# gongaa/SlidingWindowDecoder

Measured on AMD Instinct MI355X. Metric: sliding windows decoded/s, [[144,12,12]] BB p=0.003, higher is better.
Workload: dtype f64

## Files before the change

include/swd.h:

```cpp
#ifndef SWD_H
#define SWD_H

#include <stdint.h>

#ifdef __cplusplus
extern "C" {
#endif

#define SWD_ABI_VERSION 4

enum {
    SWD_EXIT_PRE = 0,
    SWD_EXIT_POST = 1,
    SWD_EXIT_OSD = 2,
    SWD_EXIT_FAIL_SET = 3,
    SWD_EXIT_FAIL_PEEL = 4,
    SWD_EXIT_NO_OSD = 5,
    SWD_EXIT_SCHED_FAULT = 6
};
#define SWD_STATUS_CONVERGE 0x100

typedef struct swd_graph_desc {
    int32_t m, n, nnz;
    const int32_t *row_ptr;
// ... 146 lines not shown
typedef struct swd_rolling swd_rolling;
swd_rolling *swd_pipeline_rolling_create(swd_pipeline *pl, int32_t max_shots);
void swd_pipeline_rolling_destroy(swd_rolling *s);
int swd_pipeline_rolling_begin(swd_rolling *s, int32_t B);
int swd_pipeline_rolling_push(swd_rolling *s, int32_t nrows, const uint8_t *det_rows, int32_t max_windows, uint8_t *faults,
                              int32_t *stats, double *min_pm, int64_t *first, int32_t *count);
int swd_pipeline_rolling_push_dev(swd_rolling *s, int32_t nrows, const uint8_t *det_rows, int64_t stride, int32_t max_windows,
                                  uint8_t *faults, int32_t *stats, double *min_pm, int64_t *first, int32_t *count, void *stream);
int swd_pipeline_rolling_finish(swd_rolling *s, int32_t nrows, const uint8_t *final_rows, uint8_t *faults, int32_t *stats,
                                double *min_pm, int32_t *shot_result);
int swd_pipeline_rolling_finish_dev(swd_rolling *s, int32_t nrows, const uint8_t *final_rows, int64_t stride, uint8_t *faults,
                                    int32_t *stats, double *min_pm, int32_t *shot_result, void *stream);
int swd_pipeline_rolling_state(swd_rolling *s, int64_t *rows_received, int64_t *windows_done, int32_t *frame_fill, int32_t *info,
                               int64_t *device_bytes);


int swd_pipeline_set_profiling(swd_pipeline *pl, int32_t on);
int swd_pipeline_get_profile(swd_pipeline *pl, int32_t B, int64_t *out);
int swd_pipeline_set_timing(swd_pipeline *pl, int32_t on);
int swd_pipeline_get_timing(swd_pipeline *pl, double *total_ms, int64_t *launches);

int swd_diag_occupy(int device, int32_t blocks, int32_t threads, int32_t lds_bytes, int32_t microseconds, void *stream);

#ifdef __cplusplus
}
#endif
#endif
```

slidingwindowdecoder_amd/_lib.py:

```python
from __future__ import annotations

import ctypes as C
import os

_HERE = os.path.dirname(os.path.abspath(__file__))
LIB_PATH = os.path.join(_HERE, os.environ.get("SWD_LIB", "libswd_hip.so"))
_lib = None


class GraphDesc(C.Structure):
    _fields_ = [("m", C.c_int32), ("n", C.c_int32), ("nnz", C.c_int32),
                ("row_ptr", C.c_void_p), ("col_idx", C.c_void_p), ("channel_probs", C.c_void_p)]


class WindowDesc(C.Structure):
    _fields_ = [("graph", GraphDesc), ("row0", C.c_int32), ("col0", C.c_int32), ("commit", C.c_int32),
                ("reserved", C.c_int32)]


class OsdwParams(C.Structure):
    _fields_ = [("pre_max_iter", C.c_int32), ("post_max_iter", C.c_int32),
                ("ms_scaling_factor", C.c_double), ("new_n", C.c_int32),
                ("osd_method", C.c_int32), ("osd_order", C.c_int32)]

# ... 57 lines not shown
    ("swd_pipeline_session_push_dev", C.c_int, [_vp, _i32, _vp, _i64, C.POINTER(_i32), C.POINTER(_i32), _vp]),
    ("swd_pipeline_session_window", C.c_int, [_vp, _i32, _vp, _vp, _vp]),
    ("swd_pipeline_session_finish", C.c_int, [_vp, _vp, _vp, _vp, _vp]),
    ("swd_pipeline_session_buffers", C.c_int, [_vp, C.POINTER(_vp), C.POINTER(_i64), C.POINTER(_i32), C.POINTER(_i32)]),
    ("swd_pipeline_rolling_create", _vp, [_vp, _i32]),
    ("swd_pipeline_rolling_destroy", None, [_vp]),
    ("swd_pipeline_rolling_begin", C.c_int, [_vp, _i32]),
    ("swd_pipeline_rolling_push", C.c_int, [_vp, _i32, _vp, _i32, _vp, _vp, _vp, C.POINTER(_i64), C.POINTER(_i32)]),
    ("swd_pipeline_rolling_push_dev", C.c_int, [_vp, _i32, _vp, _i64, _i32, _vp, _vp, _vp, C.POINTER(_i64), C.POINTER(_i32), _vp]),
    ("swd_pipeline_rolling_finish", C.c_int, [_vp, _i32, _vp, _vp, _vp, _vp, _vp]),
    ("swd_pipeline_rolling_finish_dev", C.c_int, [_vp, _i32, _vp, _i64, _vp, _vp, _vp, _vp, _vp]),
    ("swd_pipeline_rolling_state", C.c_int, [_vp, C.POINTER(_i64), C.POINTER(_i64), C.POINTER(_i32), C.POINTER(_i32), C.POINTER(_i64)]),
    ("swd_pipeline_status", C.c_int, [_vp, C.POINTER(C.c_uint32)]),
    ("swd_pipeline_set_profiling", C.c_int, [_vp, _i32]),
    ("swd_pipeline_get_profile", C.c_int, [_vp, _i32, _vp]),
    ("swd_pipeline_set_timing", C.c_int, [_vp, _i32]),
    ("swd_pipeline_get_timing", C.c_int, [_vp, C.POINTER(_dbl), C.POINTER(_i64)]),
    ("swd_sampler_create", _vp, [C.POINTER(GraphDesc), C.POINTER(GraphDesc), C.c_int]),
    ("swd_sampler_destroy", None, [_vp]),
    ("swd_sampler_info", C.c_int, [_vp, C.POINTER(_i32), C.POINTER(_i32), C.POINTER(_i32)]),
    ("swd_sampler_sample", C.c_int, [_vp, _i32, C.c_uint64, C.c_uint64, _vp, _vp, _vp]),
    ("swd_sampler_sample_dev", C.c_int, [_vp, _i32, C.c_uint64, C.c_uint64, _vp, _i64, _vp, _vp, _i64, _vp]),
    ("swd_diag_occupy", C.c_int, [C.c_int, _i32, _i32, _i32, _i32, _vp]),
]

STAT_WORDS = 8
STREAM_PACKED, STREAM_NO_STATS = 1, 2
STREAM_NO_DEPENDENCY = C.c_void_p(-1).value


def _preload_torch_hip_runtime():
    import importlib.util
    spec = importlib.util.find_spec("torch")
    if spec is None or not spec.submodule_search_locations:
        return
    libdir = os.path.join(list(spec.submodule_search_locations)[0], "lib")
    for name in ("libhsa-runtime64.so", "libamdhip64.so"):
        path = os.path.join(libdir, name)
        if os.path.exists(path):
            try:
                C.CDLL(path, mode=C.RTLD_GLOBAL)
            except OSError:
                pass


def lib():
# ... 24 lines not shown
```

slidingwindowdecoder_amd/csrc/swd_gdg_kernel.h:

```cpp
#pragma once

#define SWD_GDG_SLOTS 64
#define SWD_GDG_MAXGUESS 160
#define SWD_GDG_MAXSTEP 64
#define SWD_GDG_REC_BYTES (16 + 4 * SWD_GDG_MAXSTEP)
#define SWD_GDG_HDR_BYTES 256

__device__ __forceinline__ uint32_t ag_ld(const uint32_t *p) { return __hip_atomic_load(p, __ATOMIC_RELAXED, __HIP_MEMORY_SCOPE_AGENT); }
__device__ __forceinline__ void ag_st(uint32_t *p, uint32_t v) { __hip_atomic_store(p, v, __ATOMIC_RELAXED, __HIP_MEMORY_SCOPE_AGENT); }
__device__ __forceinline__ void ag_publish_barrier() {
    asm volatile("s_waitcnt vmcnt(0)" ::: "memory");
    __builtin_amdgcn_fence(__ATOMIC_RELEASE, "workgroup");
    __syncthreads();
}

#define SWD_ITEM_UNIT 0u
#define SWD_ITEM_SIDE 1u
#define SWD_ITEM_FINAL 2u
#define SWD_ITEM_NONE 0xFFFFFFFEu
#define SWD_ITEM_EXIT 0xFFFFFFFFu
#define SWD_GDG_ITEM_MAX_WINDOWS 256
#define SWD_GDG_ITEM_MAX_SHOTS (1 << 22)
__device__ __forceinline__ uint32_t item_unit(int b, int wi) { return (SWD_ITEM_UNIT << 30) | ((uint32_t)wi << 22) | (uint32_t)b; }
__device__ __forceinline__ uint32_t item_side(int ctxid, int slot) { return (SWD_ITEM_SIDE << 30) | ((uint32_t)ctxid << 8) | (uint32_t)slot; }
// ... 1281 lines not shown
    for (int i = 0; i < 5; ++i) R.gp[i] = 0;
#endif
    R.t[0] = wall_clock64();
    for (int l = tid; l < m; l += NT) {
        const int d = g.row_deg[l];
        s.cn_val[l] = (int8_t)(synd[g.perm[l]] ? 1 : 0);
        s.cn_deg[l] = (uint8_t)d;
        s.cn_deg0[l] = (uint8_t)d;
        s.livemask[l] = (d >= 64) ? ~0ull : ((1ull << d) - 1ull);
    }
    for (int v = tid; v < n; v += NT) { s.vn_val[v] = -1; s.hard[v] = 0; }
    for (int j = tid; j <= g.K; j += NT) s.jptr[j] = g.jptr[j];
    if (P.zero_hist)
        for (int i = tid; i < 4 * n; i += NT) hist_b[i] = 0.0;
    __syncthreads();
    GdgVC<VF, DM> vc;
    GdgCC<KG> cn;
    vn_cache_load<NT, VF, DM, true>(g, s, n, vc);
    bp_init<VF, DM>(s, vc);
    cn_cache_load<NT, KG, true>(g, s, false, s.ctid < g.m ? s.ctid : -1, 0, 1, cn);
    __syncthreads();
    int it = 0;
    R.conv = 0; R.pm = 0.0; R.pre_it = R.post_it = 0;
    R.live_vn = n; R.live_cn = m; R.live_e = g.E; R.osd_rowadds = 0;
    R.t[1] = wall_clock64();
    R.conv = bp_run<NT, VF, DM, KG, true>(g, P, s, P.pre_iter, n, vc, cn, hist_b, it, P.alpha, false);
    R.pre_it = it; R.total_it = it;
    R.t[2] = wall_clock64();
    if (R.conv) { R.exit_class = SWD_EXIT_PRE; return; }
    if (P.kind == 3) { R.exit_class = SWD_EXIT_NO_OSD; return; }

    uint64_t *key = (uint64_t *)s.scratch;
    uint16_t *idx = (uint16_t *)(s.scratch + L.off_idx);
    __syncthreads();
    if (!par || ENS) gdg_stage_graph<NT>(g_loc, g_in, s);
    for (int v = tid; v < L.npad; v += NT) {
        if (v < n) {
            const double sum = ((hist_b[v] + hist_b[n + v]) + hist_b[2 * n + v]) + hist_b[3 * n + v];
            key[v] = f2key(sum);
            idx[v] = (uint16_t)v;
        } else { key[v] = ~0ull; idx[v] = 0xFFFF; }
    }
    for (int v = tid; v < n; v += NT) G.bp_hard[v] = s.hard[v];
    __syncthreads();
    if (P.max_iter_per_step < 4)
        for (int i = P.max_iter_per_step * n + tid; i < 4 * n; i += NT) hist_b[i] = 0.0;
    int npad2 = 2;
// ... 217 lines not shown
```

slidingwindowdecoder_amd/csrc/swd_graph.h:

```cpp
#pragma once
#include <stdint.h>

#define SWD_MAX_ROW_DEG 64
#define SWD_MAX_COL_DEG 16
#define SWD_MAX_M 1024
#define SWD_MAX_E 65535
#define SWD_PAD_EDGE 0xFFFFFFFFu

struct SwdGraphDev {
    int32_t m, n, E, K, D;
    int32_t new_n, rank, wm;
    const uint16_t *jptr;
    const uint16_t *row_col;
    const uint8_t *row_deg;
    const uint16_t *perm;
    const uint16_t *iperm;
    const uint32_t *vn_edge;
    const uint16_t *vn_row;
    const uint8_t *col_deg;
    const double *llr;
    const uint16_t *vperm;
    const uint32_t *vn_edge_s;
    const double *llr_s;
};

__host__ __device__ inline uint32_t swd_edge_slot(uint32_t e) { return e & 0xFFFFu; }
__host__ __device__ inline uint32_t swd_edge_lane(uint32_t e) { return (e >> 16) & 0x3FFu; }
__host__ __device__ inline uint32_t swd_edge_j(uint32_t e) { return e >> 26; }
```

slidingwindowdecoder_amd/csrc/swd_graph.hip:

```cpp
#include <math.h>
#include <string.h>

#include <mutex>

#include "swd_host.h"

namespace swd {

static thread_local std::string g_err;

void set_error(const char *fmt, ...) {
    char buf[1024];
    va_list ap;
    va_start(ap, fmt);
    vsnprintf(buf, sizeof buf, fmt, ap);
    va_end(ap);
    g_err = buf;
}

const char *last_error() { return g_err.c_str(); }

int gf2_rank(int m, int n, const std::vector<int32_t> &row_ptr, const std::vector<int32_t> &col_idx) {
    const int W = (n + 63) / 64;
    std::vector<uint64_t> rows((size_t)m * W, 0);
// ... 24 lines not shown
            if (col_idx[e] < 0 || col_idx[e] >= n) { set_error("column index out of range in row %d", r); return -1; }
            if (e > row_ptr[r] && col_idx[e] == col_idx[e - 1]) { set_error("duplicate entry in row %d", r); return -1; }
        }
    }
    return 0;
}

void csr_transpose(int m, int n, const double *channel_probs, bool want_r2c, CsrHost &h) {
    const int E = (int)h.col_idx.size();
    h.col_ptr.assign(n + 1, 0);
    h.row_idx.resize(E);
    h.c2r.resize(E);
    std::vector<int32_t> fill(n, 0);
    for (int e = 0; e < E; ++e) h.col_ptr[h.col_idx[e] + 1]++;
    for (int v = 0; v < n; ++v) h.col_ptr[v + 1] += h.col_ptr[v];
    for (int c = 0; c < m; ++c)
        for (int e = h.row_ptr[c]; e < h.row_ptr[c + 1]; ++e) { const int v = h.col_idx[e], k = h.col_ptr[v] + fill[v]++; h.row_idx[k] = c; h.c2r[k] = e; }
    if (want_r2c) {
        h.r2c.resize(E);
        for (int k = 0; k < E; ++k) h.r2c[h.c2r[k]] = k;
    }
    h.llr.resize(n);
    for (int v = 0; v < n; ++v) h.llr[v] = log((1 - channel_probs[v]) / channel_probs[v]);
}

int Graph::build(const swd_graph_desc *g) {
    if (!g || !g->row_ptr || !g->col_idx || !g->channel_probs) { set_error("null graph description"); return -1; }
    m = g->m; n = g->n; E = g->nnz;
    if (m <= 0 || n <= 0 || E <= 0) { set_error("empty check matrix (m=%d n=%d nnz=%d)", m, n, E); return -1; }
    if (g->row_ptr[0] != 0 || g->row_ptr[m] != E) { set_error("row_ptr does not span nnz"); return -1; }
    if (m > SWD_MAX_M) { set_error("m=%d exceeds this build's limit of %d checks", m, SWD_MAX_M); return -1; }
    if (n > 65534) { set_error("n=%d exceeds this build's limit of 65534 columns", n); return -1; }
    if (E > SWD_MAX_E) { set_error("nnz=%d exceeds this build's limit of %d edges", E, SWD_MAX_E); return -1; }
    row_ptr.assign(g->row_ptr, g->row_ptr + m + 1);
    col_idx.assign(g->col_idx, g->col_idx + E);
    if (csr_check_rows(m, n, row_ptr, col_idx)) return -1;
    row_deg.assign(m, 0);
    col_deg.assign(n, 0);
    K = 0; D = 0;
    std::vector<int> cdeg(n, 0);
    for (int r = 0; r < m; ++r) {
        int d = row_ptr[r + 1] - row_ptr[r];
        if (d > SWD_MAX_ROW_DEG) { set_error("row %d has weight %d > %d", r, d, SWD_MAX_ROW_DEG); return -1; }
        if (d == 0) { set_error("row %d is empty: every check needs degree > 0 (osd_window.pyx:117)", r); return -1; }
        K = std::max(K, d);
        for (int e = row_ptr[r]; e < row_ptr[r + 1]; ++e) cdeg[col_idx[e]]++;
    }
    for (int v = 0; v < n; ++v) {
        if (cdeg[v] > SWD_MAX_COL_DEG) { set_error("column %d has weight %d > %d", v, cdeg[v], SWD_MAX_COL_DEG); return -1; }
        D = std::max(D, cdeg[v]);
        col_deg[v] = (uint8_t)cdeg[v];
    }
    perm.resize(m); iperm.resize(m);
    std::vector<int> order(m);
    for (int r = 0; r < m; ++r) order[r] = r;
    std::stable_sort(order.begin(), order.end(), [&](int a, int b) {
        return (row_ptr[a + 1] - row_ptr[a]) > (row_ptr[b + 1] - row_ptr[b]);
    });
    for (int l = 0; l < m; ++l) { perm[l] = (uint16_t)order[l]; iperm[order[l]] = (uint16_t)l; row_deg[l] = (uint8_t)(row_ptr[order[l] + 1] - row_ptr[order[l]]); }
    jptr.assign(K + 1, 0);
    for (int j = 0; j < K; ++j) {
        int cnt = 0;
        for (int l = 0; l < m; ++l) cnt += (row_deg[l] > j);
        jptr[j + 1] = (uint16_t)(jptr[j] + cnt);
    }
    row_col.assign(E, 0);
    col_ptr.assign(n + 1, 0);
    for (int v = 0; v < n; ++v) col_ptr[v + 1] = col_ptr[v] + cdeg[v];
    row_idx.assign(E, 0);
    vn_edge.assign((size_t)std::max(D, 1) * n, SWD_PAD_EDGE);
    vn_row.assign((size_t)std::max(D, 1) * n, 0xFFFF);
    std::vector<int> fill(n, 0);
    for (int r = 0; r < m; ++r) {
        const int l = iperm[r];
        for (int e = row_ptr[r]; e < row_ptr[r + 1]; ++e) {
            const int j = e - row_ptr[r];
            const int v = col_idx[e];
            const int slot = jptr[j] + l;
            row_col[slot] = (uint16_t)v;
            const int k = fill[v]++;
            row_idx[col_ptr[v] + k] = r;
            vn_edge[(size_t)k * n + v] = (uint32_t)slot | ((uint32_t)l << 16) | ((uint32_t)j << 26);
            vn_row[(size_t)k * n + v] = (uint16_t)r;
        }
    }
    llr.resize(n);
    for (int v = 0; v < n; ++v) {
        const double p = g->channel_probs[v];
        llr[v] = log((1 - p) / p);
    }
    {
        std::vector<int> ord(n);
        for (int v = 0; v < n; ++v) ord[v] = v;
        std::stable_sort(ord.begin(), ord.end(), [&](int a, int b) { return (cdeg[a] + 1) / 2 > (cdeg[b] + 1) / 2; });
        vperm.resize(n); llr_s.resize(n);
        vn_edge_s.assign((size_t)std::max(D, 1) * n, SWD_PAD_EDGE);
        for (int i = 0; i < n; ++i) {
            vperm[i] = (uint16_t)ord[i];
            llr_s[i] = llr[ord[i]];
            for (int k = 0; k < D; ++k) vn_edge_s[(size_t)k * n + i] = vn_edge[(size_t)k * n + ord[i]];
        }
    }
    rank = gf2_rank(m, n, row_ptr, col_idx);
    wm = (m + 63) / 64;
    return 0;
}

int Graph::upload() {
    auto al = [](size_t x) { return (x + 255) & ~(size_t)255; };
    size_t o_jptr = 0;
    size_t o_rowcol = al(o_jptr + jptr.size() * 2);
    size_t o_rowdeg = al(o_rowcol + row_col.size() * 2);
    size_t o_perm = al(o_rowdeg + row_deg.size());
    size_t o_iperm = al(o_perm + perm.size() * 2);
    size_t o_vnedge = al(o_iperm + iperm.size() * 2);
    size_t o_vnrow = al(o_vnedge + vn_edge.size() * 4);
    size_t o_coldeg = al(o_vnrow + vn_row.size() * 2);
    size_t o_llr = al(o_coldeg + col_deg.size());
    size_t o_vperm = al(o_llr + llr.size() * 8);
    size_t o_vnedge_s = al(o_vperm + vperm.size() * 2);
    size_t o_llr_s = al(o_vnedge_s + vn_edge_s.size() * 4);
    size_t total = al(o_llr_s + llr_s.size() * 8);
    std::vector<char> h(total, 0);
    memcpy(&h[o_jptr], jptr.data(), jptr.size() * 2);
    memcpy(&h[o_rowcol], row_col.data(), row_col.size() * 2);
    memcpy(&h[o_rowdeg], row_deg.data(), row_deg.size());
    memcpy(&h[o_perm], perm.data(), perm.size() * 2);
    memcpy(&h[o_iperm], iperm.data(), iperm.size() * 2);
    memcpy(&h[o_vnedge], vn_edge.data(), vn_edge.size() * 4);
    memcpy(&h[o_vnrow], vn_row.data(), vn_row.size() * 2);
    memcpy(&h[o_coldeg], col_deg.data(), col_deg.size());
    memcpy(&h[o_llr], llr.data(), llr.size() * 8);
    memcpy(&h[o_vperm], vperm.data(), vperm.size() * 2);
    memcpy(&h[o_vnedge_s], vn_edge_s.data(), vn_edge_s.size() * 4);
    memcpy(&h[o_llr_s], llr_s.data(), llr_s.size() * 8);
    if (dev.reserve(total)) return -1;
    SWD_HIP(hipMemcpy(dev.p, h.data(), total, hipMemcpyHostToDevice));
    char *b = (char *)dev.p;
    d.m = m; d.n = n; d.E = E; d.K = K; d.D = D; d.rank = rank; d.wm = wm; d.new_n = 0;
    d.jptr = (const uint16_t *)(b + o_jptr);
    d.row_col = (const uint16_t *)(b + o_rowcol);
    d.row_deg = (const uint8_t *)(b + o_rowdeg);
    d.perm = (const uint16_t *)(b + o_perm);
    d.iperm = (const uint16_t *)(b + o_iperm);
    d.vn_edge = (const uint32_t *)(b + o_vnedge);
    d.vn_row = (const uint16_t *)(b + o_vnrow);
    d.col_deg = (const uint8_t *)(b + o_coldeg);
    d.llr = (const double *)(b + o_llr);
    d.vperm = (const uint16_t *)(b + o_vperm);
    d.vn_edge_s = (const uint32_t *)(b + o_vnedge_s);
    d.llr_s = (const double *)(b + o_llr_s);
    return 0;
}

}

extern "C" const char *swd_last_error(void) { return swd::last_error(); }
extern "C" int swd_abi_version(void) { return SWD_ABI_VERSION; }
extern "C" int swd_device_count(void) {
    int c = 0;
    if (hipGetDeviceCount(&c) != hipSuccess) return 0;
    return c;
}
```

slidingwindowdecoder_amd/csrc/swd_host.h:

```cpp
#pragma once
#include <hip/hip_runtime.h>
#include <stdarg.h>
#include <stdint.h>
#include <stdio.h>

#include <algorithm>
#include <string>
#include <vector>

#include "swd.h"
#include "swd_graph.h"

namespace swd {

void set_error(const char *fmt, ...);

#define SWD_HIP(expr)                                                                         \
    do {                                                                                      \
        hipError_t _e = (expr);                                                               \
        if (_e != hipSuccess) {                                                               \
            swd::set_error("%s failed: %s (%s:%d)", #expr, hipGetErrorString(_e), __FILE__,   \
                           __LINE__);                                                         \
            return -1;                                                                        \
        }                                                                                     \
// ... 25 lines not shown
        p = q; cap = got;
        return 0;
    }
    template <class T> T *as() { return (T *)p; }
};

constexpr size_t SWD_STAGE_MAX = 4u << 20;
struct PinnedBuf {
    void *p = nullptr;
    size_t cap = 0;
    ~PinnedBuf() { if (p) (void)hipHostFree(p); }
    int reserve(size_t bytes) {
        if (bytes <= cap) return 0;
        if (p) (void)hipHostFree(p);
        p = nullptr; cap = 0;
        SWD_HIP(hipHostMalloc(&p, bytes, hipHostMallocDefault));
        cap = bytes;
        return 0;
    }
};

struct Graph {
    int m = 0, n = 0, E = 0, K = 0, D = 0, rank = 0, wm = 0;
    std::vector<uint16_t> jptr, row_col, perm, iperm, vn_row;
    std::vector<uint8_t> row_deg, col_deg;
    std::vector<uint32_t> vn_edge, vn_edge_s;
    std::vector<uint16_t> vperm;
    std::vector<double> llr, llr_s;
    std::vector<int32_t> row_ptr, col_idx, col_ptr, row_idx;
    DevBuf dev;
    SwdGraphDev d{};

    int build(const swd_graph_desc *g);
    int upload();
};

int gf2_rank(int m, int n, const std::vector<int32_t> &row_ptr, const std::vector<int32_t> &col_idx);

int csr_check_rows(int m, int n, const std::vector<int32_t> &row_ptr, std::vector<int32_t> &col_idx);

struct CsrHost {
    std::vector<int32_t> row_ptr, col_idx, col_ptr, row_idx, c2r, r2c;
    std::vector<double> llr;
};
void csr_transpose(int m, int n, const double *channel_probs, bool want_r2c, CsrHost &h);

}
```

slidingwindowdecoder_amd/csrc/swd_osdw.hip:

```cpp
#include <thread>

#include "swd_plan.h"
#include "swd_variants.h"

namespace swd {

int make_layout(const Graph &g, int new_n, int nt, int kind, SwdLdsLayout &L, bool big, int lds_budget) {
    const int m = g.m, n = g.n, E = g.E, wm = g.wm;
    const int npad = std::max(next_pow2(n), 2);
    L.npad = npad;
    L.off_idx = npad * 8;
    L.off_aux = align_up(npad * 10, 16);
    int osd_bytes = align_up(L.off_aux + m * wm * 8 + wm * 8 + g.rank * 4 + n * 2 + 16, 16);
    const int osd_bytes_at_aux = osd_bytes;
    L.off_oring = -1;
    if (wm <= 4 && nt >= 256 && !big) { L.off_oring = osd_bytes; osd_bytes += align_up(SWD_QUAD_RING_BYTES, 16); }
    const int kset = std::max(new_n - g.rank, 0);
    auto cs_need = [&](int cp) { return align_up(n * 2 + kset * 2 + g.rank * 4 + 64 + 8, 8) + g.rank * 8 + std::max(wm * cp, 64 + wm) * 8; };
    L.cs_par = nt;
    while (L.cs_par > std::min(nt, 256) && cs_need(L.cs_par) > npad * 8) L.cs_par -= 64;
    const int cs_bytes = cs_need(L.cs_par);
    if (cs_bytes <= npad * 8) L.off_cs = 0;
    else { L.off_cs = osd_bytes; osd_bytes += align_up(cs_bytes, 16); }
    const int rare_bytes = L.off_aux + std::max(n * 2, 3 * 256 * 4);
    int scratch = std::max(std::max((E + 1 + 2 * (nt / 64)) * 8, osd_bytes), std::max(rare_bytes, n * 2));
    L.off_cord = align_up((g.K * m * 2 <= scratch) ? std::max(L.off_aux, g.K * m * 2) : L.off_aux, 16);
    L.off_rc = align_up(std::max(L.off_cord + 66 * 4 + m * 2, L.off_aux + 3 * 256 * 4), 16);
    L.off_bak = align_up(L.off_rc + E * 2, 16);
    scratch = std::max(scratch, L.off_bak + 10 * m + 2 * n + 8);
    L.off_oslot = -1;
    if (wm > 4 && wm <= 9 && nt >= 1024) {
// ... 852 lines not shown
```

slidingwindowdecoder_amd/csrc/swd_osdw_kernel.h:

```cpp
#pragma once
#include <type_traits>
#include <hip/hip_runtime.h>
#include <stdint.h>

#include "swd.h"
#include "swd_graph.h"

#define SWD_DMAX 10

#ifndef SWD_OSDW_TUNED
#define SWD_OSDW_TUNED 0
#endif
#ifndef SWD_TUNED_NT
#define SWD_TUNED_NT 256
#endif
#define SWD_P16(NT) (SWD_OSDW_TUNED && (NT) <= SWD_TUNED_NT)
#ifndef SWD_POST_DEPTH2
#define SWD_POST_DEPTH2 0
#endif
#ifndef SWD_POST_SORTED
#define SWD_POST_SORTED 3
#endif
#ifndef SWD_POST_KGP
#define SWD_POST_KGP 0
// ... 2493 lines not shown
    if constexpr (kHyb) {
        const int cells = g.E + 1 + 2 * (NT / 64);
        const int cap = (L.off_pmsg >= 0) ? (L.pmsg_bytes - rec_b) / 8 : 0;
        const int lo = max(cells - cap, 0);
        s.msg_lo = (cap > 0) ? (uint32_t)lo << 3 : 0xFFFFFFFFu;
        s.msg_alt = (char *)s.hard - L.off_hard + (L.off_pmsg >= 0 ? L.off_pmsg + rec_b : 0);
    }
    if constexpr (kTbl) bp_init_tbl<NT, VF, DM, kHyb>(g, s);
    else bp_init<VF, DM, kHyb>(s, vc);
#ifdef SWD_INITPROF
    const long long ip3 = wall_clock64();
#endif
    std::conditional_t<SWD_P16(NT), CnCacheP<KG>, CnCacheP<KG, 3>> cn;
    if constexpr (SF) {
        const uint32_t e = cn_map[s.ctid];
        cn_cache_load<NT, KG, true>(g, s, false, (e & 0xFFFFu) == 0xFFFFu ? -1 : (int)(e & 0xFFFFu), (int)((e >> 16) & 3u), (int)(e >> 18), cn);
    } else {
        cn_cache_load<NT, KG, true>(g, s, false, s.ctid < m ? s.ctid : -1, 0, 1, cn);
    }
    __syncthreads();

    int it = 0;
    R.conv = 0; R.pm = 0.0; R.pre_it = R.post_it = 0;
    R.live_vn = n; R.live_cn = m; R.live_e = g.E; R.osd_rowadds = 0;
    uint16_t *list0 = (uint16_t *)s.scratch;
    R.t[1] = wall_clock64();
#ifdef SWD_INITPROF
    if (tid == 0) { s.scal[20] = (int)(ip0 - R.t[0]); s.scal[21] = (int)(ip1 - ip0); s.scal[22] = (int)(ip2 - ip1); s.scal[23] = (int)(ip3 - ip2); s.scal[24] = (int)(R.t[1] - ip3); }
#endif

    double hs[VF];
#pragma unroll
    for (int i = 0; i < VF; ++i) hs[i] = 0.0;
    if constexpr (kTbl) R.conv = bp_run<NT, VF, DM, KG, true, SF, HACC, false, false, kHyb, false, true>(g, P, s, P.pre_iter, n, vc, cn, hist_b, it, P.alpha, false, hs);
    else
    if (kRec && rec_on) {
        if constexpr (kRec) R.conv = bp_run<NT, VF, DM, KG, true, SF, HACC, false, false, kHyb, true>(g, P, s, P.pre_iter, n, vc, cn, hist_b, it, P.alpha, false, hs);
    } else
    R.conv = bp_run<NT, VF, DM, KG, true, SF, HACC, false, false, kHyb>(g, P, s, P.pre_iter, n, vc, cn, hist_b, it, P.alpha, false, hs);
    R.pre_it = it;
    R.t[2] = wall_clock64();
    if (R.conv) {
        R.exit_class = SWD_EXIT_PRE;
#ifdef SWD_INITPROF
        const long long pm0 = wall_clock64();
#endif
        if (want_pm) R.pm = ordered_pm<NT>(g, s, list0);
// ... 855 lines not shown
```

slidingwindowdecoder_amd/csrc/swd_plan.h:

```cpp
#pragma once
#include <string.h>

#include <map>
#include <memory>
#include <mutex>

#include <stdlib.h>

#include "swd_host.h"
#include "swd_osdw_kernel.h"

namespace swd {

inline int next_pow2(int x) { int p = 1; while (p < x) p <<= 1; return p; }
inline int align_up(int x, int a) { return (x + a - 1) / a * a; }

int make_layout(const Graph &g, int new_n, int nt, int kind, SwdLdsLayout &L, bool big = false, int lds_budget = 0);

struct WindowHost {
    std::shared_ptr<Graph> g;
    int new_n = 0, row0 = 0, col0 = 0, commit = 0;
    SwdLdsLayout L{};
};

// ... 151 lines not shown
            live_s.swap(sessions);
        }
        for (SessionBase *ss : live_s) {
            std::lock_guard<std::mutex> lk(ss->mu);
            if (ss->ev_set) (void)hipEventSynchronize(ss->ev);
            ss->plan = nullptr;
        }
        if (ev0) { (void)hipEventDestroy(ev0); (void)hipEventDestroy(ev1); }
        for (auto &sl : slot) if (sl.done) (void)hipEventDestroy(sl.done);
    }

    int add_window(const swd_graph_desc *gd, int row0, int col0, int commit,
                   std::map<std::string, std::shared_ptr<Graph>> &cache) {
        std::string key((const char *)gd->row_ptr, (size_t)(gd->m + 1) * 4);
        key.append((const char *)gd->col_idx, (size_t)gd->nnz * 4);
        key.append((const char *)gd->channel_probs, (size_t)gd->n * 8);
        WindowHost w;
        auto itc = cache.find(key);
        if (itc != cache.end()) w.g = itc->second;
        else {
            w.g = std::make_shared<Graph>();
            if (w.g->build(gd)) return -1;
            if (w.g->D > SWD_DMAX) { set_error("column weight %d exceeds this build's bound %d", w.g->D, SWD_DMAX); return -1; }
            if (w.g->upload()) return -1;
            cache[key] = w.g;
        }
        const int m = w.g->m, n = w.g->n;
        const int req_new_n = (kind == 0) ? p.new_n : gp.new_n;
        w.new_n = (req_new_n <= 0) ? std::min(n, 2 * m) : std::min(req_new_n, n);
        if (kind == 0 && p.osd_order > w.new_n - w.g->rank) {
            set_error("For this code, the OSD order should be set in the range 0<=osd_oder<=%d.", w.new_n - w.g->rank);
            return -1;
        }
        if (commit < 0 || commit > n || row0 < 0 || col0 < 0) {
            set_error("invalid window placement: row0 %d col0 %d commit %d for a window with %d columns", row0, col0, commit, n);
            return -1;
        }
        w.row0 = row0; w.col0 = col0; w.commit = commit;
        wins.push_back(w);
        return 0;
    }

    void size_snapshots() {
        snap_stride = 0;
        for (auto &w : wins) {
            const int64_t rec = ((w.new_n + 2 * w.g->m + 7) & ~7) + 8 * (int64_t)w.g->m;
            const int ens_slots = (kind == 1 && gp.multi_thread == 1) ? 2 + std::max(gp.max_side_depth - gp.max_tree_depth, 0) : 0;
            snap_stride = std::max(snap_stride, rec * (gdg_parallel ? SWD_GDG_SLOTS : std::max(std::max(max_guess, 1), ens_slots)));
        }
        snap_stride = (snap_stride + 15) & ~(int64_t)15;
    }

    int finalize(const swd_graph_desc *chk) {
        if (kind == 0 && p.osd_method == 1 && p.osd_order > 15) { set_error("osd_e supports osd_order <= 15 on the device"); return -1; }
        if (kind != 0) {
            max_guess = ((1 << gp.max_tree_depth) - 1) * 2 + gp.max_side_depth - gp.max_tree_depth;
            if (max_guess < 0) max_guess = 0;
            if (max_guess > SWD_GDG_MAXGUESS) { set_error("max_guess=%d exceeds the device limit of %d snapshots", max_guess, SWD_GDG_MAXGUESS); return -1; }
            if (gp.multi_thread == 1 && (gp.max_side_depth - gp.max_tree_depth > SWD_GDG_MAXGUESS - 2 || gp.max_tree_depth > 6)) {
                set_error("multi_thread: at most %d side threads and tree depth 6 on the device", SWD_GDG_MAXGUESS - 2); return -1;
            }
            gdg_parallel = kind == 1 && gp.multi_thread != 1 && max_guess <= SWD_GDG_SLOTS && gp.max_side_branch_step <= SWD_GDG_MAXSTEP && gp.max_step < 200 && gp.max_side_depth < 200 &&
                           wins.size() <= SWD_GDG_ITEM_MAX_WINDOWS && !getenv("SWD_GDG_SERIAL");
            for (auto &w : wins) new_n_max = std::max(new_n_max, w.new_n);
            size_snapshots();
        }
        nmax = 0;
        int lmax = 0, mmax = 0;
        dm = 0;
        for (auto &w : wins) { nmax = std::max(nmax, w.g->n); dm = std::max(dm, w.g->D); }
        int kmax = 0;
        mmax = 0;
        for (auto &w : wins) { kmax = std::max(kmax, w.g->K); mmax = std::max(mmax, w.g->m); }
// ... 21 lines not shown
            const int det_est = chk ? chk->m : mtop_rows;
            for (auto &w : wins) {
                make_layout(*w.g, w.new_n, nt, kind, w.L, big, 160 * 1024 - 64 - align_up(det_est, 16));
                lmax = std::max(lmax, w.L.total); mmax = std::max(mmax, w.row0 + w.g->m);
                big_stride = std::max<int64_t>(big_stride, align_up(w.L.big_scratch, 256));
            }
            if (chk) { num_det = chk->m; num_col = chk->n; } else { num_det = mmax; num_col = 0; }
            if (mmax > num_det) { set_error("window rows exceed the global check matrix (%d > %d)", mmax, num_det); return -1; }
            off_det = align_up(lmax, 16) + 16;
            int dmax = num_det;
            if (kind == 0 && nt <= SWD_TUNED_NT) {
                dmax = 0;
                for (auto &w : wins) dmax = std::max(dmax, std::min((w.row0 + w.g->m + 3) & ~3, (num_det + 3) & ~3) - (w.row0 & ~3));
            }
            lds_total = off_det + align_up(dmax, 16);
            if (lds_total > 160 * 1024) {
                set_error("window graph needs %d bytes of LDS per shot (> 163840)%s", lds_total, big ? " even with its messages in HBM" : "");
                variant = nullptr;
                continue;
            }
            break;
        }
        if (!variant) return -1;
        post_depth2 = kind != 0 && !getenv("SWD_GDG_NO_DEPTH2");
        for (auto &w : wins) post_depth2 = post_depth2 && w.new_n <= 2 * nt;
        if (kind == 1 && gp.multi_thread == 1) {
            const int ens_slots = 2 + std::max(gp.max_side_depth - gp.max_tree_depth, 0);
            const int vfp = (post_depth2 && vf > 2) ? 2 : vf;
            for (auto &w : wins) {
                const int64_t rec = ((w.new_n + 2 * w.g->m + 7) & ~7) + 8 * (int64_t)w.g->m;
                const int64_t cells = std::max<int64_t>(w.g->E + 1 + 2 * (nt / 64), (int64_t)vfp * variant->dm * nt);
                const int64_t forkb = ((rec + 15) & ~(int64_t)15) + ((cells * 8 + 15) & ~(int64_t)15);
                snap_stride = std::max(snap_stride, ((rec * ens_slots + 15) & ~(int64_t)15) + gp.max_tree_depth * forkb + 2 * (((int64_t)w.new_n + 15) & ~(int64_t)15) + 16);
            }
            snap_stride = (snap_stride + 15) & ~(int64_t)15;
        }
        if (status.reserve(64)) return -1;
        SWD_HIP(hipMemset(status.p, 0, 64));
        std::vector<SwdWindowDev> hw(wins.size());
        if (variant->sf) {
            std::vector<uint32_t> all, one;
            for (auto &w : wins) { split_map(*w.g, nt, 4 * variant->kg, &one); all.insert(all.end(), one.begin(), one.end()); }
            if (d_cnmap.reserve(all.size() * 4)) return -1;
            SWD_HIP(hipMemcpy(d_cnmap.p, all.data(), all.size() * 4, hipMemcpyHostToDevice));
        }
        for (size_t i = 0; i < wins.size(); ++i) {
            hw[i].cn_map = variant->sf ? d_cnmap.as<uint32_t>() + i * (size_t)nt : nullptr;
            hw[i].g = wins[i].g->d;
            hw[i].g.new_n = wins[i].new_n;
            hw[i].L = wins[i].L;
            hw[i].row0 = wins[i].row0; hw[i].col0 = wins[i].col0; hw[i].commit = wins[i].commit; hw[i].pad = 0;
        }
        if (d_wins.reserve(hw.size() * sizeof(SwdWindowDev))) return -1;
        SWD_HIP(hipMemcpy(d_wins.p, hw.data(), hw.size() * sizeof(SwdWindowDev), hipMemcpyHostToDevice));
// ... 51 lines not shown
    }
    const long long units = (long long)a.B * a.W;
    static const int grid_pct = getenv("SWD_GRID_PCT") ? std::max(1, atoi(getenv("SWD_GRID_PCT"))) : 100;
    const unsigned grid = (unsigned)std::min<long long>(units, std::max(1, slots[d->device & 63] * grid_pct / 100));
    if constexpr (KIND == 7) {
        const int Dp = d->gp.max_tree_depth, NS = std::max(d->gp.max_side_depth - d->gp.max_tree_depth, 0);
        if (!BIG && a.W > 1 && a.B < SWD_GDG_ITEM_MAX_SHOTS && a.W <= SWD_GDG_ITEM_MAX_WINDOWS && !getenv("SWD_ENS_TICKETS") && !d->stream_serial) {
            a.slot_scratch = 1;
            const bool tasks = Dp >= 1 && !getenv("SWD_ENS_NO_TASKS");
            unsigned nctx = 64;
            while (nctx < 2 * grid) nctx <<= 1;
            const int nh = 1 + ((1 << Dp) - 1) + NS, nforks = Dp >= 1 ? (1 << (Dp - 1)) : 0;
            unsigned cap = 1024;
            while (cap < (unsigned)a.B + (tasks ? nctx * (unsigned)((1 << Dp) + 2 + NS) : 0u) + 2u * grid + 1024u) cap <<= 1;
            const size_t qbytes = 16 + (size_t)cap * 8, fbytes = 16 + (size_t)nctx * 8;
            const int pos_b = align_up(d->new_n_max * 2, 16), vec_b = align_up(d->new_n_max, 16);
            a.gdgp.off_pos = SWD_GDG_HDR_BYTES; a.gdgp.off_node = a.gdgp.off_pos + pos_b; a.gdgp.off_rec = a.gdgp.off_node + align_up(std::max(nforks, 1) * 8 + NS * 12, 16);
            a.gdgp.off_err = a.gdgp.off_rec + align_up(nh * 16, 16); a.gdgp.err_stride = vec_b; a.gdgp.ens_hyps = nh;
            a.gdgp.ctx_stride = align_up(a.gdgp.off_err + (nh + 1) * vec_b, 256);
            int64_t forkb = 0, rec16 = 0;
            const int vfp = (d->post_depth2 && d->vf > 2) ? 2 : d->vf;
            for (auto &w : d->wins) {
                const int64_t rec = ((w.new_n + 2 * w.g->m + 7) & ~7) + 8 * (int64_t)w.g->m;
                const int64_t cells = std::max<int64_t>(w.g->E + 1 + 2 * (NT / 64), (int64_t)vfp * DM * NT);
                forkb = std::max(forkb, ((rec + 15) & ~(int64_t)15) + ((cells * 8 + 15) & ~(int64_t)15));
                rec16 = std::max(rec16, (rec + 15) & ~(int64_t)15);
            }
            a.gdgp.csnap_stride = ((int64_t)nforks * forkb + (int64_t)NS * rec16 + 255) & ~(int64_t)255;
            Plan::LaunchSlot &sl = *d->cur;
            if (sl.gq.reserve(qbytes)) return -1;
            a.gdgp.q = sl.gq.as<uint32_t>(); a.gdgp.qmask = cap - 1;
            a.gdgp.shots_inflight = (int)std::min<long long>(a.B, grid);
            SWD_HIP(hipMemsetAsync(a.gdgp.q, 0, qbytes, st));
            if (tasks) {
                if (sl.gfq.reserve(fbytes) || sl.gctx.reserve((size_t)nctx * a.gdgp.ctx_stride) || sl.gsnap.reserve((size_t)nctx * a.gdgp.csnap_stride + 256)) return -1;
                if (sl.gfree_n != (int)nctx) {
                    std::vector<uint64_t> tmpl(2 + nctx);
                    tmpl[0] = (uint64_t)nctx << 32; tmpl[1] = 0;
                    for (unsigned t = 0; t < nctx; ++t) tmpl[2 + t] = ((uint64_t)(t + 1) << 32) | t;
                    if (sl.gfree_tmpl.reserve(fbytes)) return -1;
                    SWD_HIP(hipMemcpy(sl.gfree_tmpl.p, tmpl.data(), fbytes, hipMemcpyHostToDevice));
                    sl.gfree_n = (int)nctx;
                }
                a.gdgp.fq = sl.gfq.as<uint32_t>(); a.gdgp.fmask = nctx - 1;
                a.gdgp.ctx = sl.gctx.as<uint8_t>(); a.gdgp.csnap = sl.gsnap.as<uint8_t>();
                a.gdgp.nctx = (int)nctx;
                SWD_HIP(hipMemcpyAsync(a.gdgp.fq, sl.gfree_tmpl.p, fbytes, hipMemcpyDeviceToDevice, st));
// ... 94 lines not shown
```

Before: 5.264 million.

## Optimize edge slot layout to reduce LDS bank conflicts with padding

```diff
diff --git a/include/swd.h b/include/swd.h
--- a/include/swd.h
+++ b/include/swd.h
@@ -192,6 +192,9 @@
 
 int swd_diag_occupy(int device, int32_t blocks, int32_t threads, int32_t lds_bytes, int32_t microseconds, void *stream);
 
+int swd_graph_layout(const swd_graph_desc *g, int32_t pads, int32_t *info, uint16_t *jptr, uint16_t *row_col, uint16_t *perm,
+                     uint16_t *iperm, uint8_t *row_deg, uint32_t *vn_edge, uint32_t *vn_edge_s, uint16_t *vperm);
+
 #ifdef __cplusplus
 }
 #endif
diff --git a/slidingwindowdecoder_amd/_lib.py b/slidingwindowdecoder_amd/_lib.py
--- a/slidingwindowdecoder_amd/_lib.py
+++ b/slidingwindowdecoder_amd/_lib.py
@@ -103,6 +103,7 @@
     ("swd_sampler_sample", C.c_int, [_vp, _i32, C.c_uint64, C.c_uint64, _vp, _vp, _vp]),
     ("swd_sampler_sample_dev", C.c_int, [_vp, _i32, C.c_uint64, C.c_uint64, _vp, _i64, _vp, _vp, _i64, _vp]),
     ("swd_diag_occupy", C.c_int, [C.c_int, _i32, _i32, _i32, _i32, _vp]),
+    ("swd_graph_layout", C.c_int, [C.POINTER(GraphDesc), _i32] + [_vp] * 9),
 ]
 
 STAT_WORDS = 8
diff --git a/slidingwindowdecoder_amd/csrc/swd_gdg_kernel.h b/slidingwindowdecoder_amd/csrc/swd_gdg_kernel.h
--- a/slidingwindowdecoder_amd/csrc/swd_gdg_kernel.h
+++ b/slidingwindowdecoder_amd/csrc/swd_gdg_kernel.h
@@ -1327,7 +1327,7 @@
     __syncthreads();
     int it = 0;
     R.conv = 0; R.pm = 0.0; R.pre_it = R.post_it = 0;
-    R.live_vn = n; R.live_cn = m; R.live_e = g.E; R.osd_rowadds = 0;
+    R.live_vn = n; R.live_cn = m; R.live_e = g.nnz; R.osd_rowadds = 0;
     R.t[1] = wall_clock64();
     R.conv = bp_run<NT, VF, DM, KG, true>(g, P, s, P.pre_iter, n, vc, cn, hist_b, it, P.alpha, false);
     R.pre_it = it; R.total_it = it;
diff --git a/slidingwindowdecoder_amd/csrc/swd_graph.h b/slidingwindowdecoder_amd/csrc/swd_graph.h
--- a/slidingwindowdecoder_amd/csrc/swd_graph.h
+++ b/slidingwindowdecoder_amd/csrc/swd_graph.h
@@ -10,6 +10,7 @@
 struct SwdGraphDev {
     int32_t m, n, E, K, D;
     int32_t new_n, rank, wm;
+    int32_t nnz, pad_;
     const uint16_t *jptr;
     const uint16_t *row_col;
     const uint8_t *row_deg;
diff --git a/slidingwindowdecoder_amd/csrc/swd_graph.hip b/slidingwindowdecoder_amd/csrc/swd_graph.hip
--- a/slidingwindowdecoder_amd/csrc/swd_graph.hip
+++ b/slidingwindowdecoder_amd/csrc/swd_graph.hip
@@ -1,4 +1,5 @@
 #include <math.h>
+#include <stdlib.h>
 #include <string.h>
 
 #include <mutex>
@@ -70,6 +71,145 @@
     }
     h.llr.resize(n);
     for (int v = 0; v < n; ++v) h.llr[v] = log((1 - channel_probs[v]) / channel_probs[v]);
+}
+
+void Graph::fill_tables() {
+    jptr.assign(K + 1, 0);
+    for (int j = 0; j < K; ++j) {
+        int cnt = 0;
+        for (int l = 0; l < m; ++l) cnt += (row_deg[l] > j);
+        jptr[j + 1] = (uint16_t)(jptr[j] + cnt + dpad[j]);
+    }
+    S = jptr[K];
+    row_col.assign(S, 0);
+    vn_edge.assign((size_t)std::max(D, 1) * n, SWD_PAD_EDGE);
+    vn_row.assign((size_t)std::max(D, 1) * n, 0xFFFF);
+    std::vector<int> fill(n, 0);
+    for (int r = 0; r < m; ++r) {
+        const int l = iperm[r];
+        for (int e = row_ptr[r]; e < row_ptr[r + 1]; ++e) {
+            const int j = epos[e];
+            const int v = col_idx[e];
+            const int slot = jptr[j] + l;
+            row_col[slot] = (uint16_t)v;
+            const int k = fill[v]++;
+            vn_edge[(size_t)k * n + v] = (uint32_t)slot | ((uint32_t)l << 16) | ((uint32_t)j << 26);
+            vn_row[(size_t)k * n + v] = (uint16_t)r;
+        }
+    }
+}
+
+void Graph::fill_listed() {
+    vn_edge_s.assign((size_t)std::max(D, 1) * n, SWD_PAD_EDGE);
+    for (int i = 0; i < n; ++i)
+        for (int k = 0; k < D; ++k) vn_edge_s[(size_t)k * n + i] = vn_edge[(size_t)k * n + vperm[i]];
+}
+
+long Graph::layout_cost(long *loads, long *stores) const {
+    long cl = 0, cs = 0;
+    for (int k = 0; k < D; ++k)
+        for (int v0 = 0; v0 < n; v0 += 16) {
+            if ((v0 & 31) == 0) {
+                int h[32] = {0}, mx = 0;
+                for (int v = v0; v < std::min(n, v0 + 32); ++v) {
+                    const uint32_t e = vn_edge[(size_t)k * n + v];
+                    if (e != SWD_PAD_EDGE) mx = std::max(mx, ++h[swd_edge_slot(e) & 31]);
+                }
+                cl += mx;
+            }
+            int h[16] = {0}, mx = 0;
+            for (int v = v0; v < std::min(n, v0 + 16); ++v) {
+                const uint32_t e = vn_edge[(size_t)k * n + v];
+                if (e != SWD_PAD_EDGE) mx = std::max(mx, ++h[swd_edge_slot(e) & 15]);
+            }
+            cs += mx;
+        }
+    if (loads) *loads = cl;
+    if (stores) *stores = cs;
+    return cl + cs;
+}
+
+void Graph::optimize_layout(int pads) {
+    if (pads < 0) pads = 0;
+    if (E + pads > SWD_MAX_E) pads = SWD_MAX_E - E;
+    std::vector<int> gl(E), gs(E), erow(E);
+    {
+        std::vector<int> fill(n, 0);
+        for (int r = 0; r < m; ++r)
+            for (int e = row_ptr[r]; e < row_ptr[r + 1]; ++e) {
+                const int v = col_idx[e];
+                const int k = fill[v]++;
+                erow[e] = r;
+                gl[e] = (v >> 5) * D + k;
+                gs[e] = (v >> 4) * D + k;
+            }
+    }
+    const int NGL = ((n + 31) >> 5) * D, NGS = ((n + 15) >> 4) * D;
+    std::vector<uint16_t> pad(K, 0);
+    for (int j = 0, left = pads; j + 1 < K && left > 0; ++j, --left) pad[j] = 1;
+    std::vector<int> jp(K + 1, 0);
+    for (int j = 0; j < K; ++j) {
+        int cnt = 0;
+        for (int l = 0; l < m; ++l) cnt += (row_deg[l] > j);
+        jp[j + 1] = jp[j] + cnt + pad[j];
+    }
+    std::vector<uint8_t> pos(epos);
+    std::vector<uint16_t> lane(iperm);
+    std::vector<int> slot(E);
+    std::vector<uint8_t> hl((size_t)NGL * 32, 0), hs((size_t)NGS * 16, 0);
+    for (int e = 0; e < E; ++e) {
+        slot[e] = jp[pos[e]] + lane[erow[e]];
+        hl[(size_t)gl[e] * 32 + (slot[e] & 31)]++;
+        hs[(size_t)gs[e] * 16 + (slot[e] & 15)]++;
+    }
+    auto mv = [&](int e, int s0, int s1) -> int {
+        uint8_t *L = &hl[(size_t)gl[e] * 32], *T = &hs[(size_t)gs[e] * 16];
+        int d = 0;
+        if ((s0 ^ s1) & 31) { d += 2 * (2 * ((int)L[s1 & 31] - (int)L[s0 & 31]) + 2); L[s0 & 31]--; L[s1 & 31]++; }
+        if ((s0 ^ s1) & 15) { d += 2 * ((int)T[s1 & 15] - (int)T[s0 & 15]) + 2; T[s0 & 15]--; T[s1 & 15]++; }
+        return d;
+    };
+    std::vector<int> run1(m), lane_row(m);
+    for (int l = 0; l < m;) { int h = l; while (h < m && row_deg[h] == row_deg[l]) ++h; for (int q = l; q < h; ++q) run1[q] = h; l = h; }
+    for (int r = 0; r < m; ++r) lane_row[lane[r]] = r;
+    const int kSweeps = 12;
+    for (int sweep = 0; sweep < kSweeps; ++sweep) {
+        long gained = 0;
+        for (int r = 0; r < m; ++r)
+            for (int a = row_ptr[r]; a < row_ptr[r + 1]; ++a)
+                for (int b = a + 1; b < row_ptr[r + 1]; ++b) {
+                    const int sa = slot[a], sb = slot[b];
+                    const int d = mv(a, sa, sb) + mv(b, sb, sa);
+                    if (d < 0 || (d == 0 && (sweep & 1))) { std::swap(pos[a], pos[b]); slot[a] = sb; slot[b] = sa; gained -= d; }
+                    else { mv(b, sa, sb); mv(a, sb, sa); }
+                }
+        for (int la = 0; la < m && (sweep & 3) == 0; ++la)
+            for (int lb = la + 1; lb < run1[la]; ++lb) {
+                const int r1 = lane_row[la], r2 = lane_row[lb];
+                int d = 0;
+                for (int e = row_ptr[r1]; e < row_ptr[r1 + 1]; ++e) d += mv(e, slot[e], slot[e] - la + lb);
+                for (int e = row_ptr[r2]; e < row_ptr[r2 + 1]; ++e) d += mv(e, slot[e], slot[e] - lb + la);
+                if (d < 0) {
+                    for (int e = row_ptr[r1]; e < row_ptr[r1 + 1]; ++e) slot[e] += lb - la;
+                    for (int e = row_ptr[r2]; e < row_ptr[r2 + 1]; ++e) slot[e] += la - lb;
+                    lane[r1] = (uint16_t)lb; lane[r2] = (uint16_t)la; lane_row[lb] = r1; lane_row[la] = r2;
+                    gained -= d;
+                } else {
+                    for (int e = row_ptr[r2]; e < row_ptr[r2 + 1]; ++e) mv(e, slot[e] - lb + la, slot[e]);
+                    for (int e = row_ptr[r1]; e < row_ptr[r1 + 1]; ++e) mv(e, slot[e] - la + lb, slot[e]);
+                }
+            }
+        if (!gained && !(sweep & 1)) break;
+    }
+    long cur = 0;
+    for (int g = 0; g < NGL; ++g) { int mx = 0; for (int b = 0; b < 32; ++b) mx = std::max(mx, (int)hl[(size_t)g * 32 + b]); cur += mx; }
+    for (int g = 0; g < NGS; ++g) { int mx = 0; for (int b = 0; b < 16; ++b) mx = std::max(mx, (int)hs[(size_t)g * 16 + b]); cur += mx; }
+    if (cur >= cost_natural) return;
+    epos = pos; iperm = lane; dpad = pad;
+    for (int r = 0; r < m; ++r) perm[iperm[r]] = (uint16_t)r;
+    fill_tables();
+    fill_listed();
+    cost = layout_cost();
 }
 
 int Graph::build(const swd_graph_desc *g) {
@@ -106,32 +246,20 @@
         return (row_ptr[a + 1] - row_ptr[a]) > (row_ptr[b + 1] - row_ptr[b]);
     });
     for (int l = 0; l < m; ++l) { perm[l] = (uint16_t)order[l]; iperm[order[l]] = (uint16_t)l; row_deg[l] = (uint8_t)(row_ptr[order[l] + 1] - row_ptr[order[l]]); }
-    jptr.assign(K + 1, 0);
-    for (int j = 0; j < K; ++j) {
-        int cnt = 0;
-        for (int l = 0; l < m; ++l) cnt += (row_deg[l] > j);
-        jptr[j + 1] = (uint16_t)(jptr[j] + cnt);
-    }
-    row_col.assign(E, 0);
+    epos.resize(E);
+    for (int r = 0; r < m; ++r)
+        for (int e = row_ptr[r]; e < row_ptr[r + 1]; ++e) epos[e] = (uint8_t)(e - row_ptr[r]);
+    dpad.assign(K, 0);
     col_ptr.assign(n + 1, 0);
     for (int v = 0; v < n; ++v) col_ptr[v + 1] = col_ptr[v] + cdeg[v];
     row_idx.assign(E, 0);
-    vn_edge.assign((size_t)std::max(D, 1) * n, SWD_PAD_EDGE);
-    vn_row.assign((size_t)std::max(D, 1) * n, 0xFFFF);
-    std::vector<int> fill(n, 0);
-    for (int r = 0; r < m; ++r) {
-        const int l = iperm[r];
-        for (int e = row_ptr[r]; e < row_ptr[r + 1]; ++e) {
-            const int j = e - row_ptr[r];
-            const int v = col_idx[e];
-            const int slot = jptr[j] + l;
-            row_col[slot] = (uint16_t)v;
-            const int k = fill[v]++;
-            row_idx[col_ptr[v] + k] = r;
-            vn_edge[(size_t)k * n + v] = (uint32_t)slot | ((uint32_t)l << 16) | ((uint32_t)j << 26);
-            vn_row[(size_t)k * n + v] = (uint16_t)r;
-        }
-    }
+    {
+        std::vector<int> fill(n, 0);
+        for (int r = 0; r < m; ++r)
+            for (int e = row_ptr[r]; e < row_ptr[r + 1]; ++e) { const int v = col_idx[e]; row_idx[col_ptr[v] + fill[v]++] = r; }
+    }
+    fill_tables();
+    cost_natural = cost = layout_cost();
     llr.resize(n);
     for (int v = 0; v < n; ++v) {
         const double p = g->channel_probs[v];
@@ -142,12 +270,8 @@
         for (int v = 0; v < n; ++v) ord[v] = v;
         std::stable_sort(ord.begin(), ord.end(), [&](int a, int b) { return (cdeg[a] + 1) / 2 > (cdeg[b] + 1) / 2; });
         vperm.resize(n); llr_s.resize(n);
-        vn_edge_s.assign((size_t)std::max(D, 1) * n, SWD_PAD_EDGE);
-        for (int i = 0; i < n; ++i) {
-            vperm[i] = (uint16_t)ord[i];
-            llr_s[i] = llr[ord[i]];
-            for (int k = 0; k < D; ++k) vn_edge_s[(size_t)k * n + i] = vn_edge[(size_t)k * n + ord[i]];
-        }
+        for (int i = 0; i < n; ++i) { vperm[i] = (uint16_t)ord[i]; llr_s[i] = llr[ord[i]]; }
+        fill_listed();
     }
     rank = gf2_rank(m, n, row_ptr, col_idx);
     wm = (m + 63) / 64;
@@ -185,7 +309,7 @@
     if (dev.reserve(total)) return -1;
     SWD_HIP(hipMemcpy(dev.p, h.data(), total, hipMemcpyHostToDevice));
     char *b = (char *)dev.p;
-    d.m = m; d.n = n; d.E = E; d.K = K; d.D = D; d.rank = rank; d.wm = wm; d.new_n = 0;
+    d.m = m; d.n = n; d.E = S; d.nnz = E; d.pad_ = 0; d.K = K; d.D = D; d.rank = rank; d.wm = wm; d.new_n = 0;
     d.jptr = (const uint16_t *)(b + o_jptr);
     d.row_col = (const uint16_t *)(b + o_rowcol);
     d.row_deg = (const uint8_t *)(b + o_rowdeg);
@@ -201,6 +325,31 @@
     return 0;
 }
 
+bool natural_layout_requested() { return getenv("SWD_NATURAL_LAYOUT") != nullptr; }
+
+}
+
+extern "C" int swd_graph_layout(const swd_graph_desc *g, int32_t pads, int32_t *info, uint16_t *jptr, uint16_t *row_col, uint16_t *perm,
+                                uint16_t *iperm, uint8_t *row_deg, uint32_t *vn_edge, uint32_t *vn_edge_s, uint16_t *vperm) {
+    swd::Graph G;
+    if (G.build(g)) return -1;
+    long nl = 0, ns = 0, cl = 0, cs = 0;
+    G.layout_cost(&nl, &ns);
+    if (!swd::natural_layout_requested()) G.optimize_layout(pads);
+    G.layout_cost(&cl, &cs);
+    if (info) {
+        const int32_t v[8] = {G.S, G.K, G.D, (int32_t)cl, (int32_t)cs, (int32_t)nl, (int32_t)ns, G.S - G.E};
+        memcpy(info, v, sizeof v);
+    }
+    if (jptr) memcpy(jptr, G.jptr.data(), G.jptr.size() * 2);
+    if (row_col) memcpy(row_col, G.row_col.data(), G.row_col.size() * 2);
+    if (perm) memcpy(perm, G.perm.data(), G.perm.size() * 2);
+    if (iperm) memcpy(iperm, G.iperm.data(), G.iperm.size() * 2);
+    if (row_deg) memcpy(row_deg, G.row_deg.data(), G.row_deg.size());
+    if (vn_edge) memcpy(vn_edge, G.vn_edge.data(), G.vn_edge.size() * 4);
+    if (vn_edge_s) memcpy(vn_edge_s, G.vn_edge_s.data(), G.vn_edge_s.size() * 4);
+    if (vperm) memcpy(vperm, G.vperm.data(), G.vperm.size() * 2);
+    return 0;
 }
 
 extern "C" const char *swd_last_error(void) { return swd::last_error(); }
diff --git a/slidingwindowdecoder_amd/csrc/swd_host.h b/slidingwindowdecoder_amd/csrc/swd_host.h
--- a/slidingwindowdecoder_amd/csrc/swd_host.h
+++ b/slidingwindowdecoder_amd/csrc/swd_host.h
@@ -71,6 +71,10 @@
 
 struct Graph {
     int m = 0, n = 0, E = 0, K = 0, D = 0, rank = 0, wm = 0;
+    int S = 0;
+    std::vector<uint8_t> epos;
+    std::vector<uint16_t> dpad;
+    long cost_natural = 0, cost = 0;
     std::vector<uint16_t> jptr, row_col, perm, iperm, vn_row;
     std::vector<uint8_t> row_deg, col_deg;
     std::vector<uint32_t> vn_edge, vn_edge_s;
@@ -81,8 +85,14 @@
     SwdGraphDev d{};
 
     int build(const swd_graph_desc *g);
+    void optimize_layout(int pads);
+    long layout_cost(long *loads = nullptr, long *stores = nullptr) const;
+    void fill_tables();
+    void fill_listed();
     int upload();
 };
+
+bool natural_layout_requested();
 
 int gf2_rank(int m, int n, const std::vector<int32_t> &row_ptr, const std::vector<int32_t> &col_idx);
 
diff --git a/slidingwindowdecoder_amd/csrc/swd_osdw.hip b/slidingwindowdecoder_amd/csrc/swd_osdw.hip
--- a/slidingwindowdecoder_amd/csrc/swd_osdw.hip
+++ b/slidingwindowdecoder_amd/csrc/swd_osdw.hip
@@ -6,7 +6,7 @@
 namespace swd {
 
 int make_layout(const Graph &g, int new_n, int nt, int kind, SwdLdsLayout &L, bool big, int lds_budget) {
-    const int m = g.m, n = g.n, E = g.E, wm = g.wm;
+    const int m = g.m, n = g.n, E = g.S, wm = g.wm;
     const int npad = std::max(next_pow2(n), 2);
     L.npad = npad;
     L.off_idx = npad * 8;
diff --git a/slidingwindowdecoder_amd/csrc/swd_osdw_kernel.h b/slidingwindowdecoder_amd/csrc/swd_osdw_kernel.h
--- a/slidingwindowdecoder_amd/csrc/swd_osdw_kernel.h
+++ b/slidingwindowdecoder_amd/csrc/swd_osdw_kernel.h
@@ -2539,7 +2539,7 @@
 
     int it = 0;
     R.conv = 0; R.pm = 0.0; R.pre_it = R.post_it = 0;
-    R.live_vn = n; R.live_cn = m; R.live_e = g.E; R.osd_rowadds = 0;
+    R.live_vn = n; R.live_cn = m; R.live_e = g.nnz; R.osd_rowadds = 0;
     uint16_t *list0 = (uint16_t *)s.scratch;
     R.t[1] = wall_clock64();
 #ifdef SWD_INITPROF
diff --git a/slidingwindowdecoder_amd/csrc/swd_plan.h b/slidingwindowdecoder_amd/csrc/swd_plan.h
--- a/slidingwindowdecoder_amd/csrc/swd_plan.h
+++ b/slidingwindowdecoder_amd/csrc/swd_plan.h
@@ -197,7 +197,6 @@
             w.g = std::make_shared<Graph>();
             if (w.g->build(gd)) return -1;
             if (w.g->D > SWD_DMAX) { set_error("column weight %d exceeds this build's bound %d", w.g->D, SWD_DMAX); return -1; }
-            if (w.g->upload()) return -1;
             cache[key] = w.g;
         }
         const int m = w.g->m, n = w.g->n;
@@ -224,6 +223,40 @@
             snap_stride = std::max(snap_stride, rec * (gdg_parallel ? SWD_GDG_SLOTS : std::max(std::max(max_guess, 1), ens_slots)));
         }
         snap_stride = (snap_stride + 15) & ~(int64_t)15;
+    }
+
+    int layout_graphs(int lmax) {
+        std::vector<Graph *> uniq;
+        for (auto &w : wins)
+            if (std::find(uniq.begin(), uniq.end(), w.g.get()) == uniq.end()) uniq.push_back(w.g.get());
+        if (!big && !natural_layout_requested()) {
+            const int tail = lds_total - align_up(lmax, 16);
+            const int limit = std::min(align_up(lds_total, 1280), 160 * 1024);
+            for (Graph *g : uniq) {
+                int pads = (kind == 0) ? std::min(g->K - 1, SWD_MAX_E - g->E) : 0;
+                for (; pads > 0; --pads) {
+                    bool ok = true;
+                    g->S = g->E + pads;
+                    for (auto &w : wins) {
+                        if (w.g.get() != g) continue;
+                        SwdLdsLayout L{};
+                        make_layout(*g, w.new_n, nt, kind, L);
+                        ok = ok && align_up(L.total, 16) + tail <= limit && (nt > SWD_TUNED_NT || L.total <= 65536) &&
+                             L.off_lslot == w.L.off_lslot && L.post_lds == w.L.post_lds && L.off_cord == w.L.off_cord && L.off_rc == w.L.off_rc &&
+                             L.off_cs == w.L.off_cs && L.cs_par == w.L.cs_par && L.off_oring == w.L.off_oring && L.off_oslot == w.L.off_oslot;
+                    }
+                    if (ok) break;
+                }
+                g->S = g->E;
+                g->optimize_layout(pads);
+            }
+            for (auto &w : wins) { make_layout(*w.g, w.new_n, nt, kind, w.L); lmax = std::max(lmax, w.L.total); }
+            off_det = align_up(lmax, 16) + 16;
+            lds_total = align_up(lmax, 16) + tail;
+        }
+        for (Graph *g : uniq)
+            if (g->upload()) return -1;
+        return 0;
     }
 
     int finalize(const swd_graph_desc *chk) {
@@ -291,6 +324,7 @@
             break;
         }
         if (!variant) return -1;
+        if (layout_graphs(lmax)) return -1;
         post_depth2 = kind != 0 && !getenv("SWD_GDG_NO_DEPTH2");
         for (auto &w : wins) post_depth2 = post_depth2 && w.new_n <= 2 * nt;
         if (kind == 1 && gp.multi_thread == 1) {
@@ -298,7 +332,7 @@
             const int vfp = (post_depth2 && vf > 2) ? 2 : vf;
             for (auto &w : wins) {
                 const int64_t rec = ((w.new_n + 2 * w.g->m + 7) & ~7) + 8 * (int64_t)w.g->m;
-                const int64_t cells = std::max<int64_t>(w.g->E + 1 + 2 * (nt / 64), (int64_t)vfp * variant->dm * nt);
+                const int64_t cells = std::max<int64_t>(w.g->S + 1 + 2 * (nt / 64), (int64_t)vfp * variant->dm * nt);
                 const int64_t forkb = ((rec + 15) & ~(int64_t)15) + ((cells * 8 + 15) & ~(int64_t)15);
                 snap_stride = std::max(snap_stride, ((rec * ens_slots + 15) & ~(int64_t)15) + gp.max_tree_depth * forkb + 2 * (((int64_t)w.new_n + 15) & ~(int64_t)15) + 16);
             }
@@ -396,7 +430,7 @@
             const int vfp = (d->post_depth2 && d->vf > 2) ? 2 : d->vf;
             for (auto &w : d->wins) {
                 const int64_t rec = ((w.new_n + 2 * w.g->m + 7) & ~7) + 8 * (int64_t)w.g->m;
-                const int64_t cells = std::max<int64_t>(w.g->E + 1 + 2 * (NT / 64), (int64_t)vfp * DM * NT);
+                const int64_t cells = std::max<int64_t>(w.g->S + 1 + 2 * (NT / 64), (int64_t)vfp * DM * NT);
                 forkb = std::max(forkb, ((rec + 15) & ~(int64_t)15) + ((cells * 8 + 15) & ~(int64_t)15));
                 rec16 = std::max(rec16, (rec + 15) & ~(int64_t)15);
             }
```

Result: faster. 5.357 million, median of 6 (+1.8%).
